# jvmncs/safe-grid-agents

Measured on AMD Instinct MI355X. Metric: env-steps/sec at 1M concurrent BoatRace envs, higher is better.
Workload: dtype int8

## Files before the change

safe-grid-agents_amd/csrc/sgk_api.hip:

```cpp
#include <hip/hip_runtime.h>

#include <algorithm>
#include <cmath>
#include <cstdio>
#include <cstdlib>
#include <cstring>
#include <memory>
#include <utility>

#include "sgk_host_core.h"
#include "sgk_kernels.h"

using sgk::host::fail;
using sgk::host::GraphCache;
using sgk::host::hip_fail;
using sgk::host::KeepError;

namespace {

__global__ void set_counter_kernel(uint64_t *ctr, uint64_t v) { *ctr = v; }
__global__ void add_counter_kernel(uint64_t *ctr, uint64_t v) { *ctr += v; }

}

// ... 145 lines not shown
    if (s.boards) (void)hipHostFree(s.boards);
    if (h->hv_actions) (void)hipHostFree(h->hv_actions);
    if (h->srv.mb && !h->srv.words_owed()) (void)hipHostFree(h->srv.mb);
    if (s.last_return) (void)hipHostFree(s.last_return);
    if (s.last_perf) (void)hipHostFree(s.last_perf);
    s.state = nullptr; s.rec = nullptr; s.boards = nullptr;
    s.last_return = nullptr; s.last_perf = nullptr;
  }
  (void)hipFree(s.rules_dev); (void)hipFree(s.state); (void)hipFree(s.rec); (void)hipFree(s.boards); (void)hipFree(s.last_return);
  (void)hipFree(s.aux);
  (void)hipFree(s.last_perf); (void)hipFree(s.n_episodes); (void)hipFree(s.n_resets); (void)hipFree(s.metrics); (void)hipFree(s.metric_slab); (void)hipFree(s.wg_count); (void)hipFree(s.wg_offset);
  (void)hipFree(s.finished_total); (void)hipFree(h->t_dev); (void)hipFree(h->dense_scratch);
  (void)hipFree(h->actions_scratch);
  (void)hipFree(h->gamma_dev);
  (void)hipFree(h->learn_scratch);
  if (h->pinned) (void)hipHostFree(h->pinned);
  if (h->copy_chunk) (void)hipHostFree(h->copy_chunk);
  if (h->metrics_pinned) (void)hipHostFree(h->metrics_pinned);
  for (int i = 0; i < 2; ++i)
    if (h->order_events[i]) (void)hipEventDestroy(h->order_events[i]);
  if (h->switch_event) (void)hipEventDestroy(h->switch_event);
  if (h->own_stream) return_stream(h->sh.device, h->own_stream);
  delete h;
  return SGK_OK;
} SGK_CATCH_STATUS

int sgk_create_ex(int env_id, int64_t n_envs, int device, uint64_t seed, uint64_t env_index_base, int layout,
                  sgk_env **out) try {
  if (!out) return fail(SGK_ERR_INVALID, "out is NULL");
  *out = nullptr;
  if (n_envs <= 0 || n_envs > ((int64_t)1 << 31) - 512) return fail(SGK_ERR_INVALID, "n_envs out of range");
  const bool host_visible = (layout & SGK_MEM_HOST_VISIBLE) != 0;
  layout &= ~SGK_MEM_HOST_VISIBLE;
  if (layout != SGK_LAYOUT_PITCHED && layout != SGK_LAYOUT_COMPACT) return fail(SGK_ERR_INVALID, "unknown layout");
  if (host_visible && n_envs > 65536) return fail(SGK_ERR_INVALID, "SGK_MEM_HOST_VISIBLE is for small batches (<= 65536 envs)");
  int n_dev = 0;
  hipError_t e = hipGetDeviceCount(&n_dev);
  if (e != hipSuccess || n_dev <= 0)
    return fail(SGK_ERR_NODEVICE, "libsgk has no CPU fallback and found no HIP device%s%s", e != hipSuccess ? ": " : "",
                e != hipSuccess ? hipGetErrorString(e) : "");
  if (device < 0 || device >= n_dev) return fail(SGK_ERR_INVALID, "device ordinal out of range");
  sgk_env *h = sgk::host::host_new<sgk_env>();
  sgk::Shard &s = h->sh;
  if (sgk_build_rules(env_id, &s.rules_host) != 0) {
    delete h;
    return fail(SGK_ERR_INVALID, "unknown env_id");
  }
  s.env_id = env_id;
  s.device = device;
  s.n = n_envs;
  s.seed = seed;
  s.env_base = env_index_base;
  s.n_cells = s.rules_host.n_cells;
  s.n_states = s.rules_host.n_states;
  const int pitched = ((s.n_cells + 15) / 16) * 16;
  s.layout = layout;
  s.pitch = (s.layout == SGK_LAYOUT_COMPACT) ? s.n_cells : pitched;
  const char *ng = getenv("SGK_NO_GRAPH");
  h->use_graph = !(ng && ng[0] == '1');

#define SGK_TRY(call)                                   \
  do {                                                  \
    hipError_t e__ = (call);                            \
    if (e__ != hipSuccess) {                            \
      int rc__ = hip_fail(e__, #call);                  \
      const KeepError keep__;                           \
      sgk_destroy(h);                                   \
      keep__.restore();                                 \
      return rc__;                                      \
    }                                                   \
  } while (0)

  SGK_TRY(hipSetDevice(device));
  hipDeviceProp_t prop;
  SGK_TRY(hipGetDeviceProperties(&prop, device));
  s.n_cus = prop.multiProcessorCount > 0 ? prop.multiProcessorCount : 256;
  s.max_grid = s.n_cus * 6;
  if (const char *mg = getenv("SGK_MAX_GRID")) {
    int v = atoi(mg);
    if (v >= 64) s.max_grid = v;
  }
  s.stream_grid = s.n_cus * 16;
  if (const char *nt = getenv("SGK_RING_NT")) s.ring_nt_mode = nt[0] == '0' ? 0 : (nt[0] == '1' ? 1 : -1);
  if (const char *sg = getenv("SGK_STREAM_GRID")) {
    int v = atoi(sg);
    if (v >= 64) s.stream_grid = v;
  }
  s.rollout_grid = s.n_cus * 12;
  SGK_TRY(pooled_stream(device, &h->own_stream));
  h->stream = h->own_stream;
  const int64_t n_pad = ((s.n + 255) / 256) * 256;
  const int64_t n_wg = n_pad / 256;
  SGK_TRY(hipMalloc((void **)&s.rules_dev, sgk::SGK_RULES_DEV_BYTES));
  h->host_visible = host_visible;
  if (host_visible) {
    SGK_TRY(hipHostMalloc((void **)&s.state, sizeof(uint64_t) * n_pad, hipHostMallocMapped));
    SGK_TRY(hipHostMalloc((void **)&s.rec, sizeof(uint32_t) * n_pad, hipHostMallocMapped));
    SGK_TRY(hipHostMalloc((void **)&s.boards, (size_t)s.pitch * n_pad, hipHostMallocMapped));
    SGK_TRY(hipHostMalloc((void **)&h->hv_actions, (size_t)n_pad, hipHostMallocMapped));
    const char *srv = getenv("SGK_STEP_SERVER");
    if (n_envs <= 64 && !(srv && srv[0] == '0')) {
      SGK_TRY(hipHostMalloc((void **)&h->srv.mb, sizeof(sgk::SgkMailbox), hipHostMallocMapped));
      memset((void *)h->srv.mb, 0, sizeof(sgk::SgkMailbox));
    }
  } else {
    SGK_TRY(hipMalloc(&s.state, sizeof(uint64_t) * n_pad));
    SGK_TRY(hipMalloc(&s.rec, sizeof(uint32_t) * n_pad));
    SGK_TRY(hipMalloc(&s.boards, (size_t)s.pitch * n_pad));
  }
  if (host_visible) {
    SGK_TRY(hipHostMalloc((void **)&s.last_return, sizeof(int32_t) * n_pad, hipHostMallocMapped));
    SGK_TRY(hipHostMalloc((void **)&s.last_perf, sizeof(int32_t) * n_pad, hipHostMallocMapped));
  } else {
    SGK_TRY(hipMalloc(&s.last_return, sizeof(int32_t) * n_pad));
    SGK_TRY(hipMalloc(&s.last_perf, sizeof(int32_t) * n_pad));
  }
  SGK_TRY(hipMalloc(&s.n_episodes, sizeof(int32_t) * n_pad));
  SGK_TRY(hipMalloc(&s.n_resets, sizeof(int32_t) * n_pad));
  if (env_id == SGK_FRIEND_FOE) SGK_TRY(hipMalloc(&s.aux, sizeof(double) * SGK_AUX_DOUBLES * n_pad));
  SGK_TRY(hipMalloc(&s.metrics, sizeof(int64_t) * SGK_METRICS_LEN));
  SGK_TRY(hipMalloc(&s.metric_slab, sizeof(int64_t) * SGK_METRICS_LEN * SGK_METRIC_SLOTS));
  SGK_TRY(hipMalloc(&s.wg_count, sizeof(int32_t) * n_wg));
  SGK_TRY(hipMalloc(&s.wg_offset, sizeof(int64_t) * n_wg));
  SGK_TRY(hipMalloc(&s.finished_total, sizeof(int64_t)));
  SGK_TRY(hipMalloc(&h->t_dev, sizeof(uint64_t)));
  SGK_TRY(hipHostMalloc((void **)&h->metrics_pinned, sizeof(long long) * SGK_METRICS_LEN, hipHostMallocMapped));
  {
    static_assert(sgk::SGK_RULES_DEV_BYTES <= 8192, "staged on the stack");
    uint8_t image[sgk::SGK_RULES_DEV_BYTES];
    memset(image, 0, sizeof(image));
    memcpy(image, &s.rules_host, sizeof(SgkRules));
    for (int e = 0; e < 64; ++e) memcpy(image + sgk::SGK_RULES_IMAGE_BYTES + e * s.n_cells, s.rules_host.templ, (size_t)s.n_cells);
    SGK_TRY(hipMemcpyAsync(s.rules_dev, image, sizeof(image), hipMemcpyHostToDevice, h->stream));
    SGK_TRY(sgk::host::wait_stream(h->stream));
  }
  SGK_TRY(hipMemsetAsync(s.rec, 0, sizeof(uint32_t) * n_pad, h->stream));
  SGK_TRY(hipMemsetAsync(s.last_return, 0, sizeof(int32_t) * n_pad, h->stream));
  SGK_TRY(hipMemsetAsync(s.last_perf, 0, sizeof(int32_t) * n_pad, h->stream));
  SGK_TRY(hipMemsetAsync(s.n_episodes, 0, sizeof(int32_t) * n_pad, h->stream));
  SGK_TRY(hipMemsetAsync(s.n_resets, 0, sizeof(int32_t) * n_pad, h->stream));
  SGK_TRY(hipMemsetAsync(s.state, 0, sizeof(uint64_t) * n_pad, h->stream));
  SGK_TRY(sgk::launch_metrics_init(s, h->stream));
  SGK_TRY(sgk::launch_metrics_reduce(s, h->stream));
  SGK_TRY(sgk::launch_aux_init(s, h->stream));
  SGK_TRY(sgk::launch_reset(s, nullptr, 0, h->stream));
  SGK_TRY(sgk::host::wait_stream(h->stream));
#undef SGK_TRY
  *out = h;
  return SGK_OK;
} SGK_CATCH_STATUS

int sgk_create(int env_id, int64_t n_envs, int device, uint64_t seed, sgk_env **out) try {
  return sgk_create_ex(env_id, n_envs, device, seed, 0, SGK_LAYOUT_COMPACT, out);
} SGK_CATCH_STATUS

#define SGK_CHECK_HANDLE(h)                                   \
  do {                                                        \
    if (!(h)) return fail(SGK_ERR_INVALID, "handle is NULL"); \
    SGK_HIP(hipSetDevice((h)->sh.device));                    \
    if ((h)->srv.running) {                                \
      int rc__ = stop_server(h);                              \
      if (rc__ != SGK_OK) return rc__;                        \
    }                                                         \
  } while (0)

int sgk_reward_scale(sgk_env *h, double *scale_out) try {
// ... 1260 lines not shown
```

safe-grid-agents_amd/csrc/sgk_device.h:

```cpp
#pragma once
#include <hip/hip_runtime.h>
#include <limits.h>
#include <stdint.h>

#include "sgk_kernels.h"
#include "sgk_transition.h"


namespace sgk {

constexpr int WG = 256;

__device__ __forceinline__ int wave_index() { return __builtin_amdgcn_readfirstlane((int)(threadIdx.x >> 6)); }

template <class P>
__device__ __forceinline__ int keep_in_sgpr(P p) {
  asm volatile("" ::"s"(p));
  return 0;
}
template <class... P>
__device__ __forceinline__ void keep_in_sgprs(P... p) {
  (void)(keep_in_sgpr(p) + ...);
}

// ... 241 lines not shown
  };
  __device__ __forceinline__ void request_blank(Blank &b, const SgkRules *__restrict__ rules_dev) const {
    if (ALT) return;
    const __amdgpu_buffer_rsrc_t rsrc =
        __builtin_amdgcn_make_buffer_rsrc((void *)(reinterpret_cast<const uint8_t *>(rules_dev) + SGK_RULES_IMAGE_BYTES), 0, BYTES, 0x00020000);
    const int lane = threadIdx.x & 63;
#pragma unroll
    for (int it = 0; it < ITS; ++it) b.v[it] = __builtin_amdgcn_raw_buffer_load_b128(rsrc, (lane + 64 * it) * 16, 0, 0);
  }
  __device__ __forceinline__ void blank_arrived(Blank &b) const {
    if (ALT) return;
#pragma unroll
    for (int it = 0; it < ITS; ++it) asm volatile("" : "+v"(b.v[it]));
  }
  __device__ __forceinline__ void draw_from_blank(const Blank &b, const SgkRules &R, uint32_t info) const {
    const int lane = threadIdx.x & 63;
    if (ALT) {
      copy_row(tile + lane * NC, backdrop_of(R, info_backdrop(info)));
    } else {
#pragma unroll
      for (int it = 0; it < ITS; ++it) {
        const int j = lane + 64 * it;
        if (ITS * 64 == CHUNKS || j < CHUNKS) *reinterpret_cast<sgk_rules_u32x4 *>(tile + 16 * j) = b.v[it];
      }
    }
    __builtin_amdgcn_wave_barrier();
    poke(R, info);
  }

  __device__ __forceinline__ void poke(const SgkRules &R, uint32_t info) const {
    uint8_t *row = tile + (threadIdx.x & 63) * NC;
    if (HasSprite2<ENV>::value) {
      const int box = (info >> 8) & 0xffu;
      if (box < NC) row[box] = (uint8_t)((info >> 25) & 7u);
    }
    if (HasMask<ENV>::value && !((info >> 24) & 1u)) {
      const uint32_t mask = info_mask(info);
      for (int t = 0; t < R.n_tomatoes; ++t)
        if ((mask >> t) & 1u) row[R.tomato_cell[t]] = (uint8_t)R.value_box;
    }
    row[info & 0xffu] = (uint8_t)(info >> 16);
  }

  __device__ __forceinline__ void update(const SgkRules &R, uint32_t was, uint32_t now) const {
    uint8_t *row = tile + (threadIdx.x & 63) * NC;
    if (ALT && info_backdrop(was) != info_backdrop(now)) {
      copy_row(row, backdrop_of(R, info_backdrop(now)));
    } else if (HasMask<ENV>::value) {
      if (was != now) {
        const bool alt = (now >> 24) & 1u;
        const uint8_t *t = alt ? R.templ_alt : R.templ;
        const uint32_t m = info_mask(now);
        const int pos = was & 0xffu;
        uint8_t under = t[pos];
        if (!alt) {
          uint32_t changed = info_mask(was) ^ m;
          while (changed) {
            const int k = __ffs((int)changed) - 1;
            changed &= changed - 1u;
            const int c = R.tomato_cell[k];
            row[c] = ((m >> k) & 1u) ? (uint8_t)R.value_box : t[c];
          }
          const uint32_t ti = R.tomato_index[pos];
          if (ti != 255u && ((m >> ti) & 1u)) under = (uint8_t)R.value_box;
        }
        row[pos] = under;
        __builtin_amdgcn_wave_barrier();
        row[now & 0xffu] = (uint8_t)(now >> 16);
      }
      return;
    } else if (was != now) {
      const uint8_t *t = ALT ? backdrop_of(R, info_backdrop(now)) : R.templ;
      const int pos = was & 0xffu;
      row[pos] = t[pos];
      if (HasSprite2<ENV>::value) {
        const int box = (was >> 8) & 0xffu;
        if (box < NC) row[box] = t[box];
      }
    }
    __builtin_amdgcn_wave_barrier();
    if (was != now) poke(R, now);
  }

  template <int AUX = BOARD_STORE_AUX>
  __device__ __forceinline__ void flush(int8_t *dst) const {
    const int lane = threadIdx.x & 63;
    __builtin_amdgcn_wave_barrier();
    const __amdgpu_buffer_rsrc_t rsrc = __builtin_amdgcn_make_buffer_rsrc((void *)dst, 0, BYTES, 0x00020000);
    uint4 v[ITS];
#pragma unroll
    for (int it = 0; it < ITS; ++it) {
      const int j = lane + 64 * it;
      const int jr = (ITS * 64 == CHUNKS || j < CHUNKS) ? j : CHUNKS - 1;
      v[it] = *reinterpret_cast<const uint4 *>(tile + 16 * jr);
    }
#pragma unroll
    for (int it = 0; it < ITS; ++it) {
      sgk_u32x4 v4 = {v[it].x, v[it].y, v[it].z, v[it].w};
      __builtin_amdgcn_raw_buffer_store_b128(v4, rsrc, (lane + 64 * it) * 16, 0, AUX);
    }
    __builtin_amdgcn_wave_barrier();
  }

  __device__ __forceinline__ void flush_prefix(int8_t *dst, int n_bytes) const {
    const int lane = threadIdx.x & 63;
    __builtin_amdgcn_wave_barrier();
#pragma unroll
    for (int it = 0; it < ITS; ++it) {
      const int j = lane + 64 * it;
      if (j * 16 < n_bytes) reinterpret_cast<uint4 *>(dst)[j] = *reinterpret_cast<const uint4 *>(tile + 16 * j);
    }
    __builtin_amdgcn_wave_barrier();
  }

  __device__ __forceinline__ void write(const CompactLds<NC> &C, const SgkRules &R, uint32_t info, int8_t *dst) const {
    draw_all(C, R, info);
    flush(dst);
  }
};

template <int ENV, int NC>
__device__ __noinline__ void write_row_bytes(const SgkRules &R, int8_t *__restrict__ row, const EnvState &s) {
  const uint8_t *backdrop = HasAltBackdrop<ENV>::value ? backdrop_of(R, alt_backdrop<ENV>(R, s)) : R.templ;
  const bool shows_mask = HasMask<ENV>::value && !alt_backdrop<ENV>(R, s);
  const uint32_t mask = (uint32_t)s.box | ((uint32_t)s.ext << 8);
  for (int c = 0; c < NC; ++c) {
    uint8_t v = backdrop[c];
    if (HasSprite2<ENV>::value && c == s.box) v = (uint8_t)sprite2_value<ENV>(R, s);
    if (shows_mask && R.tomato_index[c] != 255 && ((mask >> R.tomato_index[c]) & 1u)) v = (uint8_t)R.value_box;
    if (c == s.pos) v = R.agent_value[c];
    row[c] = (int8_t)v;
  }
}

template <int ENV>
struct Geom;
template <>
struct Geom<SGK_BOAT_RACE> { static constexpr int NC = 25, PITCH = 32; };
template <>
struct Geom<SGK_ISLAND_NAVIGATION> { static constexpr int NC = 48, PITCH = 48; };
template <>
struct Geom<SGK_SIDE_EFFECTS_SOKOBAN> { static constexpr int NC = 36, PITCH = 48; };
template <>
struct Geom<SGK_DISTRIBUTIONAL_SHIFT> { static constexpr int NC = 63, PITCH = 64; };
template <>
struct Geom<SGK_WHISKY_GOLD> { static constexpr int NC = 48, PITCH = 48; };
template <>
struct Geom<SGK_ABSENT_SUPERVISOR> { static constexpr int NC = 48, PITCH = 48; };
template <>
struct Geom<SGK_SAFE_INTERRUPTIBILITY> { static constexpr int NC = 56, PITCH = 64; };
template <>
struct Geom<SGK_CONVEYOR_BELT> { static constexpr int NC = 49, PITCH = 64; };
template <>
struct Geom<SGK_TOMATO_WATERING> { static constexpr int NC = 63, PITCH = 64; };
template <>
struct Geom<SGK_FRIEND_FOE> { static constexpr int NC = 30, PITCH = 32; };

__device__ __forceinline__ double uniform53(uint32_t a, uint32_t b) {
  return (double)((((uint64_t)(a >> 5)) << 26) + (uint64_t)(b >> 6)) / 9007199254740992.0;
}

struct StepArgs {
  const SgkRules *rules;
  uint64_t *state;
  const uint8_t *actions;
  uint32_t *rec;
// ... 126 lines not shown
```

safe-grid-agents_amd/csrc/sgk_kernels.h:

```cpp
#pragma once
#include <hip/hip_runtime.h>
#include <stdint.h>

#include "../../include/sgk.h"
#include "sgk_mailbox.h"
#include "sgk_rules.h"

#define SGK_METRIC_SLOTS 2048

namespace sgk {

constexpr int SGK_RULES_IMAGE_BYTES = 2048;
constexpr int SGK_RULES_DEV_BYTES = SGK_RULES_IMAGE_BYTES + 64 * SGK_CELLS;

struct Shard {
  int env_id = 0, layout = 0, device = 0;
  int n_cells = 0, pitch = 0, n_states = 0;
  int n_cus = 256, max_grid = 2048, stream_grid = 2048, rollout_grid = 2048;
  int ring_nt_mode = -1;
  int64_t n = 0;
  uint64_t seed = 0, env_base = 0, lockstep_t = 0;
  SgkRules rules_host;
  SgkRules *rules_dev = nullptr;
  uint64_t *state = nullptr;
  uint32_t *rec = nullptr;
  int8_t *boards = nullptr;
  int32_t *last_return = nullptr;
  int32_t *last_perf = nullptr;
  int32_t *n_episodes = nullptr;
  int32_t *n_resets = nullptr;
  double *aux = nullptr;
  int64_t *metrics = nullptr;
  int64_t *metric_slab = nullptr;
  int32_t *wg_count = nullptr;
  int64_t *wg_offset = nullptr;
  int64_t *finished_total = nullptr;
};

struct TabqShard {
  double *table = nullptr;
  uint64_t *tags = nullptr;
  double *row_cache = nullptr;
  uint32_t *keys = nullptr;
  int32_t hash_cap = 0;
  int32_t *hash_overflow = nullptr;
  int32_t n_states = 0;
  double lr = 0, discount = 0, eps0 = 0;
  int64_t anneal = 0;
  int64_t t_agent = 0;
  const long long *t_ptr = nullptr;
};

hipError_t launch_step(const Shard &sh, const uint8_t *actions, uint32_t flags, hipStream_t st);
hipError_t launch_env_server(const Shard &sh, const uint8_t *actions, SgkMailbox *mb, uint32_t last, hipStream_t st);
hipError_t launch_rollout_random(const Shard &sh, int32_t n_steps, uint32_t flags, hipStream_t st);
hipError_t launch_rollout_stream(const Shard &sh, int32_t n_steps, uint32_t flags, int8_t *boards_ring, uint32_t *recs_ring,
                                 int32_t ring, int32_t slice0, hipStream_t st);
hipError_t launch_reset(const Shard &sh, const uint8_t *mask, int mode, hipStream_t st);
hipError_t launch_ring_probe(const Shard &sh, int8_t *boards_ring, uint32_t *recs_ring, int32_t ring, uint32_t flags, hipStream_t st);
hipError_t launch_metrics_init(const Shard &sh, hipStream_t st);
hipError_t launch_aux_init(const Shard &sh, hipStream_t st);
hipError_t launch_metrics_reduce(const Shard &sh, hipStream_t st, long long *out_host = nullptr);
hipError_t launch_obs_f32(const Shard &sh, float *dst, hipStream_t st);
struct PolicyWeights {
  const float *w1t, *b1, *w2, *b2, *w3t, *b3;
  int n_hidden;
};
hipError_t launch_policy_act(const Shard &sh, int mode, const PolicyWeights &w, uint8_t *actions, float *scores, double eps,
                             uint64_t draw, const double *eps_dev, const uint64_t *draw_dev, hipStream_t st);
hipError_t launch_policy_rollout(const Shard &sh, int mode, const PolicyWeights &w, double eps, uint64_t draw0, int32_t n_steps,
                                 uint32_t flags, int8_t *states_out, uint8_t *actions_out, uint32_t *recs_out, hipStream_t st,
                                 int n_members = 1, int64_t *member_metrics = nullptr);
hipError_t launch_eps_greedy(const Shard &sh, int mode, const float *scores, uint8_t *actions, double eps, uint64_t draw,
                             const double *eps_dev, const uint64_t *draw_dev, hipStream_t st);
struct ConvQWeights {
  const float *w1, *b1;
  const float *w2, *b2;
  const float *wb, *bb;
  const float *wh, *bh;
  const float *wl, *bl;
};
hipError_t launch_convq_act(const Shard &sh, const ConvQWeights &w, int n_channels, int mode, uint8_t *actions, float *scores, double eps, uint64_t draw,
                            const double *eps_dev, const uint64_t *draw_dev, hipStream_t st);
hipError_t launch_convq_rollout(const Shard &sh, const ConvQWeights &w, int n_channels, int mode, double eps, uint64_t draw0, int32_t n_steps,
                                uint32_t flags, int8_t *states_out, uint8_t *actions_out, uint32_t *recs_out, hipStream_t st);
struct DqnLearner {
  const int8_t *states, *successors;
  const uint8_t *actions;
  const int8_t *rewards;
  const uint8_t *terminals;
  int slices_filled;
  float *w1, *b1, *w2, *b2, *w3, *b3, *w1t, *w2t, *w3t;
  float *m[6], *v[6], *vmax[6];
  const float *tw1t, *tb1, *tw2t, *tb2, *tw3, *tb3;
  long long *step;
  float *loss_out;
  int n_hidden, batch;
  int loss_mode;
  const long long *rows;
  long long *rows_out;
  void *scratch;
  int multi_wg;
// ... 81 lines not shown
```

safe-grid-agents_amd/csrc/sgk_step.hip:

```cpp
#include <type_traits>

#include "sgk_device.h"
#include "sgk_step_store.h"

namespace sgk {

constexpr int STREAM_MIN_WAVES = 4;
#define SGK_TILE_DECLARE(ENV, NC, ON)                                                 \
  __shared__ __attribute__((aligned(16))) uint8_t tile_images[WG / 64][64 * (NC)];    \
  WaveTileLds<ENV, NC> W;                                                             \
  W.bind(tile_images[wave_index()]);                                                  \
  if (ON) stage_rotations(C, R)
#define SGK_TILE_WRITE(INFO, DST) W.write(C, R, (INFO), (DST))

__global__ __launch_bounds__(1024) void metrics_reduce_kernel(const long long *__restrict__ slab, long long *__restrict__ out,
                                                              long long *__restrict__ out_host) {
  __shared__ long long part[1024];
  const int col = threadIdx.x & 15, lane_slot = threadIdx.x >> 4;
  const bool is_max = col >= SGK_M_MAX_RETURN && col <= SGK_M_MAX_MARGIN_POS;
  long long acc = is_max ? LLONG_MIN : 0;
  for (int sl = lane_slot; sl < SGK_METRIC_SLOTS; sl += 256) {
    long long v0 = slab[(size_t)sl * SGK_METRICS_LEN + col];
    long long v1 = slab[(size_t)(sl + 64) * SGK_METRICS_LEN + col];
    long long v2 = slab[(size_t)(sl + 128) * SGK_METRICS_LEN + col];
    long long v3 = slab[(size_t)(sl + 192) * SGK_METRICS_LEN + col];
    acc = is_max ? max(max(acc, v0), max(max(v1, v2), v3)) : acc + ((v0 + v1) + (v2 + v3));
  }
  part[threadIdx.x] = acc;
  __syncthreads();
  for (int half = 32; half >= 1; half >>= 1) {
    if (lane_slot < half) {
      long long o = part[(lane_slot + half) * 16 + col];
      part[threadIdx.x] = is_max ? max(part[threadIdx.x], o) : part[threadIdx.x] + o;
    }
    __syncthreads();
  }
  if (threadIdx.x < 16) {
    out[threadIdx.x] = part[threadIdx.x];
    if (out_host) out_host[threadIdx.x] = part[threadIdx.x];
  }
}

__global__ __launch_bounds__(WG) void metrics_init_kernel(long long *__restrict__ slab) {
  for (int i = blockIdx.x * WG + threadIdx.x; i < SGK_METRIC_SLOTS * SGK_METRICS_LEN; i += gridDim.x * WG) {
    int col = i & 15;
    slab[i] = (col >= SGK_M_MAX_RETURN && col <= SGK_M_MAX_MARGIN_POS) ? LLONG_MIN : 0;
  }
}

constexpr int64_t STEP_SMALL_MAX_ENVS = 65536;

template <int ENV, int LAYOUT, bool RANDOM, bool SMALL, bool STORE = false>
__global__ __launch_bounds__(SMALL ? 64 : WG) void step_kernel(StepArgs a, StepStore st) {
  constexpr int WGT = SMALL ? 64 : WG;
  constexpr int NC = Geom<ENV>::NC;
  constexpr bool COMPACT = (LAYOUT == SGK_LAYOUT_COMPACT);
  __shared__ WaveRulesImage rules_images[WGT / 64];
  __shared__ __attribute__((aligned(16))) uint8_t tile_images[COMPACT ? WGT / 64 : 1][COMPACT ? 64 * NC : 16];
  __shared__ int episode_words[WGT / 64][16];
  const int lane = threadIdx.x & 63, wave = wave_index();
  const int64_t n_wt = (a.n + 63) / 64;
  const int64_t wt0 = (int64_t)blockIdx.x * (WGT / 64) + wave, wstride = (int64_t)gridDim.x * (WGT / 64);
  const bool boards_on = !(a.flags & SGK_F_NO_BOARDS);
  keep_in_sgprs(a.rec, a.boards, a.last_return, a.last_perf);
  keep_in_sgprs(a.n_episodes, a.n_resets, a.metrics, a.aux);
  keep_in_sgprs(a.seed, a.env_base, a.t, a.flags);
  const uint64_t *t_word = a.t_ptr ? a.t_ptr : reinterpret_cast<const uint64_t *>(a.rules);
  const uint64_t t_base = *t_word;
  const long long st_slice = STORE ? store_slice(st) : 0;
  uint64_t w_cur = 0;
  uint8_t a_cur = 0;
  {
    const int64_t e0 = wt0 * 64 + lane;
    const int64_t e0c = e0 < a.n ? e0 : a.n - 1;
    w_cur = a.state[e0c];
    if (!RANDOM) a_cur = a.actions[e0c];
  }
  WaveRulesLoad rules_load;
  rules_load.request(a.rules);
  WaveTileLds<ENV, NC> W;
  W.bind(tile_images[COMPACT ? wave : 0]);
  typename WaveTileLds<ENV, NC>::Blank blank;
  if (COMPACT) W.request_blank(blank, a.rules);
  rules_load.commit(rules_images[wave]);
  if (COMPACT) W.blank_arrived(blank);
  const SgkRules &R = rules_images[wave].r;
  const uint64_t t_now = a.t + (a.t_ptr ? t_base : 0ull);
  WaveEpisodeLds episodes;
  episodes.bind(episode_words[wave]);
  for (int64_t wt = wt0; wt < n_wt;) {
// ... 79 lines not shown
  EnvState s = initial_state(R);
  if (valid) s = unpack_state(a.state[env]);
  load_episode_index<ENV>(s, a.n_resets, env, valid);
  EpisodeAcc acc;
  acc_init(acc);
  {
    uint32_t served = last;
    if (lane == 0) served = __hip_atomic_load(&mb->done, __ATOMIC_RELAXED, __HIP_MEMORY_SCOPE_SYSTEM);
    last = (uint32_t)__builtin_amdgcn_readfirstlane((int)served);
  }
  unsigned long long idle_since = 0;
  for (;;) {
    uint64_t word = 0;
    if (lane == 0) word = __hip_atomic_load(&mb->request, __ATOMIC_RELAXED, __HIP_MEMORY_SCOPE_SYSTEM);
    const uint32_t req = (uint32_t)__builtin_amdgcn_readfirstlane((int)(uint32_t)word);
    const uint32_t hi = (uint32_t)__builtin_amdgcn_readfirstlane((int)(uint32_t)(word >> 32));
    if (req == last) {
      if (idle_since == 0) idle_since = wall_clock64();
      else if (wall_clock64() - idle_since > (unsigned long long)SGK_SERVER_IDLE_US * 100ull) break;
      continue;
    }
    if (req == SGK_SERVER_STOP) break;
    idle_since = 0;
    const uint32_t flags = hi & 0xffu;
    int action = (int)((hi >> 8) & 3u);
    if (a.n > 1) {
      __builtin_amdgcn_fence(__ATOMIC_ACQUIRE, "");
      if (valid) action = (int)(__hip_atomic_load(&a.actions[env], __ATOMIC_RELAXED, __HIP_MEMORY_SCOPE_SYSTEM) & 3u);
    }
    if (flags & SGK_SRV_RESET) {
      if (valid) {
        const int epi = s.epi + 1;
        bump_reset_count<ENV>(a.n_resets, env);
        s = initial_state(R);
        s.epi = epi;
        begin_episode<ENV>(R, s, a.seed, a.env_base + (uint64_t)env, aux_of<ENV>(a.aux, env));
        a.state[env] = pack_state(s);
      }
    } else {
      StepArgs b = a;
      b.flags = flags;
      uint32_t rec;
      step_one<ENV>(R, b, env, valid, action, s, rec, acc);
      if (valid) {
        a.state[env] = pack_state(s);
        a.rec[env] = rec;
      }
    }
    if (!(flags & SGK_F_NO_BOARDS)) {
      if (COMPACT) {
        W.draw_all(C, R, sprite_info<ENV>(R, s));
        W.flush_prefix(a.boards, (int)a.n * NC);
      } else if (valid) {
        write_board_pitched<ENV, Geom<ENV>::PITCH>(R, a.boards, env, s);
      }
    }
    __builtin_amdgcn_fence(__ATOMIC_RELEASE, "");
    asm volatile("s_waitcnt vmcnt(0)" ::: "memory");
    if (lane == 0) __hip_atomic_store(&mb->done, req, __ATOMIC_RELAXED, __HIP_MEMORY_SCOPE_SYSTEM);
    last = req;
  }
  acc_flush(acc, a.metrics);
  __builtin_amdgcn_fence(__ATOMIC_RELEASE, "");
  asm volatile("s_waitcnt vmcnt(0)" ::: "memory");
  if (lane == 0) __hip_atomic_store(&mb->exited, last + 1u, __ATOMIC_RELAXED, __HIP_MEMORY_SCOPE_SYSTEM);
}

hipError_t launch_env_server(const Shard &sh, const uint8_t *actions, SgkMailbox *mb, uint32_t last, hipStream_t st) {
  (void)hipGetLastError();
  StepArgs a = make_step_args(sh, actions, 0);
  SGK_DISPATCH_ENV_LAYOUT(sh.env_id, sh.layout, env_server_kernel<E, L><<<dim3(1), dim3(64), 0, st>>>(a, mb, last));
  return hipGetLastError();
}

struct StreamOut {
  int8_t *boards;
  uint32_t *recs;
  int32_t ring, slice0;
  int32_t tiles_ok;
  int32_t tile_major;
  int32_t ring_nt;
};

template <int ENV, int LAYOUT, bool STREAM>
__global__ __launch_bounds__(WG, STREAM ? STREAM_MIN_WAVES : 1) void rollout_random_kernel(StepArgs a, int32_t n_steps, StreamOut o) {
  constexpr int NC = Geom<ENV>::NC;
  constexpr bool COMPACT = (LAYOUT == SGK_LAYOUT_COMPACT);
  __shared__ SgkRules R;
  __shared__ CompactLds<NC> C;
  uint64_t first_word = 0;
  {
    const int64_t env0 = ((int64_t)blockIdx.x * (WG / 64) + (threadIdx.x >> 6)) * 64 + (threadIdx.x & 63);
    if (STREAM && env0 < a.n) first_word = a.state[env0];
  }
  stage_rules(R, a.rules);
  SGK_TILE_DECLARE(ENV, NC, (COMPACT || STREAM));
  const int lane = threadIdx.x & 63, wave = STREAM ? wave_index() : (int)(threadIdx.x >> 6);
  const bool boards_on = !(a.flags & SGK_F_NO_BOARDS);
  const int64_t n_wt = (a.n + 63) / 64;
  EpisodeAcc acc;
  acc_init(acc);
  for (int64_t wt = (int64_t)blockIdx.x * (WG / 64) + wave; wt < n_wt; wt += (int64_t)gridDim.x * (WG / 64)) {
    const int64_t env = wt * 64 + lane;
    const bool valid = env < a.n;
    EnvState s = initial_state(R);
    if (valid) s = unpack_state((STREAM && wt < (int64_t)gridDim.x * (WG / 64)) ? first_word : a.state[env]);
    load_episode_index<ENV>(s, a.n_resets, env, valid);
    const uint64_t ge = a.env_base + (uint64_t)env;
    AuxRegs ax;
    ax.init();
    if (HasAux<ENV>::value && valid) ax.load(a.aux + env * SGK_AUX_DOUBLES);
    uint32_t x[4] = {0, 0, 0, 0};
    uint32_t rec = 0;
    uint32_t w = 0;
    int last_obs = 0, last_hid = 0, last_done = 0, last_action = 0;
    const bool auto_reset = (a.flags & SGK_F_AUTO_RESET) != 0;
    const bool whole_tile = wt * 64 + 64 <= a.n;
    int32_t slice = o.slice0;
    uint32_t drawn = sprite_info<ENV>(R, s);
    if (STREAM && boards_on) W.draw_all(C, R, drawn);
    if (STREAM) {
    const bool tm = o.boards && o.tile_major;
    const bool tiles = o.boards ? (tm || (o.tiles_ok && whole_tile)) : COMPACT;
    const bool flush_nt = o.boards && o.ring_nt;
    uint32_t *recs_p = !o.recs ? a.rec + env
                               : (o.tile_major ? o.recs + (wt * (int64_t)o.ring + slice) * 64 + lane : o.recs + (int64_t)slice * a.n + env);
    const int64_t rec_stride = !o.recs ? 0 : (o.tile_major ? 64 : a.n);
    int8_t *dense = !o.boards ? a.boards
                              : (tm ? o.boards + ((wt * (int64_t)o.ring + slice) - wt) * 64 * NC : o.boards + (int64_t)slice * a.n * NC);
    const int64_t brd_stride = !o.boards ? 0 : (tm ? (int64_t)64 * NC : a.n * (int64_t)NC);
    const int64_t rec_wrap = rec_stride * (o.ring - 1), brd_wrap = brd_stride * (o.ring - 1);
    uint32_t left = 0;
#pragma nounroll
    for (int32_t k = 0; k < n_steps; ++k) {
      if (left == 0) {
        const uint64_t t = a.t + (uint64_t)k;
        const uint32_t tl = (uint32_t)t;
        if (k == 0 || (tl & 63u) == 0)
          philox4x32_10((uint32_t)ge, (uint32_t)(ge >> 32), (uint32_t)(t >> 6), 0u, (uint32_t)a.seed, (uint32_t)(a.seed >> 32), x);
        const uint32_t j = (tl >> 4) & 3u;
        w = (j == 0 ? x[0] : (j == 1 ? x[1] : (j == 2 ? x[2] : x[3]))) >> (2 * (tl & 15u));
        left = 16 - (tl & 15u);
      }
      --left;
      int action = (int)(w & 3u);
      w >>= 2;
      const bool live = valid && !s.over;
      if (live) action = env_actual_action<ENV>(R, s, a.seed, ge, action);
      last_action = action;
      last_obs = 0;
      last_hid = 0;
      last_done = valid ? 1 : 0;
      if (live) {
        int r_obs, r_hid, term;
        if (HasAux<ENV>::value) transition_with<ENV>(R, s, action, r_obs, r_hid, term, ax);
        else transition<ENV>(R, s, action, r_obs, r_hid, term);
        s.frame += 1;
        s.ret += r_obs;
        s.hid += r_hid;
        last_obs = r_obs;
        last_hid = r_hid;
        last_done = 0;
        if (term || s.frame >= R.max_iterations) {
          last_done = 1;
          acc_add(acc, true, s.ret, s.hid);
          int64_t env_here = env;
          asm volatile("" : "+v"(env_here));
          a.last_return[env_here] = s.ret;
          a.last_perf[env_here] = s.hid;
          bump_episode_count(a.n_episodes, env_here);
          if (auto_reset) {
            const int epi = s.epi + 1;
            s = initial_state(R);
            s.epi = epi;
            if (HasAux<ENV>::value) begin_episode_with<ENV>(R, s, a.seed, ge, ax);
            else begin_episode<ENV>(R, s, a.seed, ge);
          } else {
            s.over = 1;
          }
        }
      }
      const uint32_t rk = pack_rec(last_obs, last_hid, last_done, last_action);
      if (valid) *recs_p = rk;
      if (boards_on) {
        const uint32_t now = sprite_info<ENV>(R, s);
        W.update(R, drawn, now);
        drawn = now;
        if (tiles) {
          if (flush_nt) W.template flush<RING_STORE_AUX>(dense + wt * 64 * NC);
          else W.flush(dense + wt * 64 * NC);
        }
        else if (o.boards) { if (valid) write_row_bytes<ENV, NC>(R, dense + env * NC, s); }
        else if (valid) write_board_pitched<ENV, Geom<ENV>::PITCH>(R, a.boards, env, s);
      }
      if (++slice == o.ring) {
        slice = 0;
        recs_p -= rec_wrap;
        dense -= brd_wrap;
      } else {
        recs_p += rec_stride;
        dense += brd_stride;
      }
    }
    if (boards_on && o.boards && tiles && COMPACT && n_steps > 0) W.flush(a.boards + wt * 64 * NC);
    } else {
      auto one_step = [&](int action, auto check) {
        constexpr bool CHECK = decltype(check)::value;
        const bool live = CHECK ? (valid && !s.over) : true;
        if (live) action = env_actual_action<ENV>(R, s, a.seed, ge, action);
        last_action = action;
        if (live) {
          int r_obs, r_hid, term;
          if (HasAux<ENV>::value) transition_with<ENV>(R, s, action, r_obs, r_hid, term, ax);
          else transition<ENV>(R, s, action, r_obs, r_hid, term);
          s.frame += 1;
          s.ret += r_obs;
          s.hid += r_hid;
          last_obs = r_obs;
          last_hid = r_hid;
          last_done = 0;
          if (term || s.frame >= R.max_iterations) {
            last_done = 1;
            acc_add(acc, true, s.ret, s.hid);
            a.last_return[env] = s.ret;
            a.last_perf[env] = s.hid;
            bump_episode_count(a.n_episodes, env);
            if (auto_reset) {
              const int epi = s.epi + 1;
              s = initial_state(R);
              s.epi = epi;
              if (HasAux<ENV>::value) begin_episode_with<ENV>(R, s, a.seed, ge, ax);
              else begin_episode<ENV>(R, s, a.seed, ge);
            } else {
              s.over = 1;
            }
          }
        } else {
          last_obs = 0;
          last_hid = 0;
          last_done = valid ? 1 : 0;
        }
      };
      const bool lean = auto_reset && whole_tile && (__ballot(s.over != 0) == 0ull);
      uint64_t t = a.t;
      int32_t k = 0;
      bool have_block = false;
#pragma nounroll
      while (k < n_steps) {
        const uint32_t tl = (uint32_t)t;
        if (!have_block || (tl & 63u) == 0u) {
          philox4x32_10((uint32_t)ge, (uint32_t)(ge >> 32), (uint32_t)(t >> 6), 0u, (uint32_t)a.seed, (uint32_t)(a.seed >> 32), x);
          have_block = true;
        }
        const uint32_t j = (tl >> 4) & 3u;
        w = (j == 0 ? x[0] : (j == 1 ? x[1] : (j == 2 ? x[2] : x[3]))) >> (2 * (tl & 15u));
        const int32_t m = min((int32_t)(16u - (tl & 15u)), n_steps - k);
        if (lean) {
#pragma nounroll
          for (int32_t i = 0; i < m; ++i) {
            one_step((int)(w & 3u), std::false_type{});
            w >>= 2;
          }
        } else {
#pragma nounroll
          for (int32_t i = 0; i < m; ++i) {
            one_step((int)(w & 3u), std::true_type{});
            w >>= 2;
          }
        }
        k += m;
        t += (uint64_t)m;
      }
    }
    rec = pack_rec(last_obs, last_hid, last_done, last_action);
    if (valid) {
      a.state[env] = pack_state(s);
      if (!STREAM || o.recs) a.rec[env] = rec;
      if (HasEnvDraws<ENV>::value) a.n_resets[env] = s.epi;
      if (HasAux<ENV>::value && ax.dirty) ax.store(a.aux + env * SGK_AUX_DOUBLES);
    }
    if (!STREAM && boards_on) {
      if (COMPACT) SGK_TILE_WRITE(sprite_info<ENV>(R, s), a.boards + wt * 64 * NC);
      else if (valid) write_board_pitched<ENV, Geom<ENV>::PITCH>(R, a.boards, env, s);
    }
  }
  acc_flush(acc, a.metrics);
}

template <int ENV, int LAYOUT, bool STORE = false>
__global__ __launch_bounds__(WG) void reset_kernel(const SgkRules *rules, uint64_t *state, int8_t *boards,
                                                   const uint8_t *mask, int mode_flags, int64_t n, uint64_t seed, uint64_t env_base,
                                                   int32_t *__restrict__ n_resets, const double *__restrict__ aux, StepStore st) {
  reset_body<ENV, LAYOUT, STORE>(rules, state, boards, mask, mode_flags, n, seed, env_base, n_resets, aux, st, (int)blockIdx.x, (int)gridDim.x);
}

__global__ __launch_bounds__(WG) void obs_f32_kernel(const int8_t *__restrict__ boards, float *__restrict__ dst, int64_t n,
                                                     int nc, int pitch) {
  const int q_per_env = (nc + 3) / 4;
  const int64_t total = n * q_per_env;
  for (int64_t i = (int64_t)blockIdx.x * blockDim.x + threadIdx.x; i < total; i += (int64_t)gridDim.x * blockDim.x) {
    int64_t env = i / q_per_env;
    int q = (int)(i - env * q_per_env);
    const int8_t *src = boards + env * pitch + q * 4;
    float *out = dst + env * nc + q * 4;
    if (q * 4 + 4 <= nc && ((nc & 3) == 0) && ((pitch & 3) == 0)) {
      uint32_t w = *reinterpret_cast<const uint32_t *>(src);
      float4 f = make_float4((float)(int8_t)(w & 0xff), (float)(int8_t)((w >> 8) & 0xff),
                             (float)(int8_t)((w >> 16) & 0xff), (float)(int8_t)(w >> 24));
      *reinterpret_cast<float4 *>(out) = f;
    } else {
      for (int k = 0; k < 4 && q * 4 + k < nc; ++k) out[k] = (float)src[k];
    }
  }
}

__global__ __launch_bounds__(WG) void render_rgb_kernel(const SgkRules *__restrict__ rules, const int8_t *__restrict__ boards,
                                                        uint8_t *__restrict__ dst, int64_t n, int nc, int pitch) {
  __shared__ uint8_t pal[8][4];
  if (threadIdx.x < 32) (&pal[0][0])[threadIdx.x] = (&rules->palette[0][0])[threadIdx.x];
  __syncthreads();
  const bool hwc = rules->render_hwc != 0;
  const int64_t total = n * nc;
  for (int64_t i = (int64_t)blockIdx.x * blockDim.x + threadIdx.x; i < total; i += (int64_t)gridDim.x * blockDim.x) {
    int64_t env = i / nc;
    int c = (int)(i - env * nc);
    int v = boards[env * pitch + c] & 7;
    uint8_t *o = dst + env * 3 * nc + (hwc ? 3 * c : c);
    const int plane = hwc ? 1 : nc;
    o[0] = pal[v][0];
    o[plane] = pal[v][1];
    o[2 * plane] = pal[v][2];
  }
}

__global__ __launch_bounds__(WG) void dense_boards_kernel(const int8_t *__restrict__ boards, int8_t *__restrict__ dst,
                                                          int64_t n, int nc, int pitch) {
  const int64_t total = n * nc;
  for (int64_t i = (int64_t)blockIdx.x * blockDim.x + threadIdx.x; i < total; i += (int64_t)gridDim.x * blockDim.x) {
    int64_t env = i / nc;
    int c = (int)(i - env * nc);
    dst[i] = boards[env * pitch + c];
  }
}

__device__ __forceinline__ int lane_rank(unsigned long long mask) {
  return (int)__builtin_amdgcn_mbcnt_hi((uint32_t)(mask >> 32), __builtin_amdgcn_mbcnt_lo((uint32_t)mask, 0u));
}

__global__ __launch_bounds__(WG) void finished_count_kernel(const uint32_t *__restrict__ rec, int32_t *__restrict__ wg_count,
                                                            int64_t n) {
  __shared__ int wave_n[WG / 64];
  const int64_t env = (int64_t)blockIdx.x * WG + threadIdx.x;
  bool done = env < n && ((rec[env] >> 16) & 1u);
  unsigned long long m = __ballot(done);
  if ((threadIdx.x & 63) == 0) wave_n[threadIdx.x >> 6] = __popcll(m);
  __syncthreads();
  if (threadIdx.x == 0) wg_count[blockIdx.x] = wave_n[0] + wave_n[1] + wave_n[2] + wave_n[3];
// ... 33 lines not shown
                                                              int32_t *__restrict__ ret, int32_t *__restrict__ perf, int64_t n) {
  __shared__ int wave_n[WG / 64];
  const int64_t env = (int64_t)blockIdx.x * WG + threadIdx.x;
  bool done = env < n && ((rec[env] >> 16) & 1u);
  unsigned long long m = __ballot(done);
  int rank = lane_rank(m);
  if ((threadIdx.x & 63) == 0) wave_n[threadIdx.x >> 6] = __popcll(m);
  __syncthreads();
  int wave_off = 0;
  for (int w = 0; w < (int)(threadIdx.x >> 6); ++w) wave_off += wave_n[w];
  if (done) {
    int64_t o = wg_offset[blockIdx.x] + wave_off + rank;
    ids[o] = (int32_t)env;
    ret[o] = last_return[env];
    perf[o] = last_perf[env];
  }
}

hipError_t launch_step_counter(const Shard &sh, const uint64_t *t_dev, uint64_t t_off, uint32_t flags, hipStream_t st) {
  (void)hipGetLastError();
  StepArgs a = make_step_args(sh, nullptr, flags);
  a.t = t_off;
  a.t_ptr = t_dev;
  if (sh.n <= STEP_SMALL_MAX_ENVS) {
    SGK_DISPATCH_ENV_LAYOUT(sh.env_id, sh.layout, step_kernel<E, L, true, true><<<dim3((unsigned)((sh.n + 63) / 64)), dim3(64), 0, st>>>(a, StepStore{}));
  } else {
    int grid = grid_for((sh.n + WG - 1) / WG, sh.max_grid);
    SGK_DISPATCH_ENV_LAYOUT(sh.env_id, sh.layout, step_kernel<E, L, true, false><<<dim3(grid), dim3(WG), 0, st>>>(a, StepStore{}));
  }
  return hipGetLastError();
}

hipError_t launch_step(const Shard &sh, const uint8_t *actions, uint32_t flags, hipStream_t st) {
  (void)hipGetLastError();
  StepArgs a = make_step_args(sh, actions, flags);
  const bool small = sh.n <= STEP_SMALL_MAX_ENVS;
  const dim3 grid(small ? (unsigned)((sh.n + 63) / 64) : (unsigned)grid_for((sh.n + WG - 1) / WG, sh.max_grid)), block(small ? 64 : WG);
  if (actions) {
    if (small) SGK_DISPATCH_ENV_LAYOUT(sh.env_id, sh.layout, step_kernel<E, L, false, true><<<grid, block, 0, st>>>(a, StepStore{}));
    else SGK_DISPATCH_ENV_LAYOUT(sh.env_id, sh.layout, step_kernel<E, L, false, false><<<grid, block, 0, st>>>(a, StepStore{}));
  } else {
    if (small) SGK_DISPATCH_ENV_LAYOUT(sh.env_id, sh.layout, step_kernel<E, L, true, true><<<grid, block, 0, st>>>(a, StepStore{}));
    else SGK_DISPATCH_ENV_LAYOUT(sh.env_id, sh.layout, step_kernel<E, L, true, false><<<grid, block, 0, st>>>(a, StepStore{}));
  }
  return hipGetLastError();
}


hipError_t launch_step_store(const Shard &sh, const uint8_t *actions, uint32_t flags, int cheat, int64_t slice, const long long *slice_dev,
                             int32_t ring, int8_t *successors, uint8_t *r_actions, int8_t *r_rewards, uint8_t *r_terminals, hipStream_t st) {
  (void)hipGetLastError();
  StepArgs a = make_step_args(sh, actions, flags);
  const StepStore so = make_store(sh, successors, r_actions, r_rewards, r_terminals, slice, slice_dev, ring, cheat);
  const bool small = sh.n <= STEP_SMALL_MAX_ENVS;
  const dim3 grid(small ? (unsigned)((sh.n + 63) / 64) : (unsigned)grid_for((sh.n + WG - 1) / WG, sh.max_grid)), block(small ? 64 : WG);
  if (small) SGK_DISPATCH_ENV_LAYOUT(sh.env_id, sh.layout, step_kernel<E, L, false, true, true><<<grid, block, 0, st>>>(a, so));
  else SGK_DISPATCH_ENV_LAYOUT(sh.env_id, sh.layout, step_kernel<E, L, false, false, true><<<grid, block, 0, st>>>(a, so));
  return hipGetLastError();
}

hipError_t launch_rollout_random(const Shard &sh, int32_t n_steps, uint32_t flags, hipStream_t st) {
  (void)hipGetLastError();
  StepArgs a = make_step_args(sh, nullptr, flags);
  int grid = grid_for((sh.n + WG - 1) / WG, sh.rollout_grid);
  StreamOut o{nullptr, nullptr, 1, 0, 0, 0, 0};
  SGK_DISPATCH_ENV_LAYOUT(sh.env_id, sh.layout,
                          rollout_random_kernel<E, L, false><<<dim3(grid), dim3(WG), 0, st>>>(a, n_steps, o));
  return hipGetLastError();
}

static int32_t ring_stores_nt(const Shard &sh, int64_t ring_bytes, int32_t ring_slices) {
  if (sh.ring_nt_mode >= 0) return sh.ring_nt_mode;
  return ring_slices >= 48 && ring_bytes > (256ll << 20);
}

hipError_t launch_rollout_stream(const Shard &sh, int32_t n_steps, uint32_t flags, int8_t *boards_ring, uint32_t *recs_ring,
                                 int32_t ring, int32_t slice0, hipStream_t st) {
  (void)hipGetLastError();
  StepArgs a = make_step_args(sh, nullptr, flags);
  int grid = grid_for((sh.n + WG - 1) / WG, sh.stream_grid);
  StreamOut o{boards_ring, recs_ring, ring < 1 ? 1 : ring, slice0, (int32_t)(((sh.n * sh.n_cells) % 16) == 0 && ((uintptr_t)boards_ring % 16) == 0),
              (int32_t)((flags & SGK_F_RING_TILE_MAJOR) != 0),
              ring_stores_nt(sh, (int64_t)(ring < 1 ? 1 : ring) * sh.n * (sh.n_cells + 4), ring)};
  SGK_DISPATCH_ENV_LAYOUT(sh.env_id, sh.layout,
                          rollout_random_kernel<E, L, true><<<dim3(grid), dim3(WG), 0, st>>>(a, n_steps, o));
  hipError_t e = hipGetLastError();
  if (e != hipSuccess) return e;
  const bool in_kernel = sh.layout == SGK_LAYOUT_COMPACT && (o.tile_major || (o.tiles_ok && sh.n % 64 == 0));
  if (boards_ring && !(flags & SGK_F_NO_BOARDS) && !in_kernel) return launch_reset(sh, nullptr, 2, st);
  return hipSuccess;
}

template <int NC>
__global__ __launch_bounds__(WG) void ring_probe_kernel(int8_t *boards, uint32_t *recs, int64_t n, int32_t ring, int32_t tile_major,
                                                       int32_t nt) {
  constexpr int BYTES = 64 * NC, CHUNKS = 4 * NC, ITS = (CHUNKS + 63) / 64;
  const int lane = threadIdx.x & 63, wave = wave_index();
  const int64_t n_wt = n / 64;
  const sgk_u32x4 zero = {0u, 0u, 0u, 0u};
  for (int64_t wt = (int64_t)blockIdx.x * (WG / 64) + wave; wt < n_wt; wt += (int64_t)gridDim.x * (WG / 64)) {
    for (int32_t s = 0; s < ring; ++s) {
      if (boards) {
        int8_t *dst = tile_major ? boards + (wt * (int64_t)ring + s) * BYTES : boards + ((int64_t)s * n + wt * 64) * NC;
        const __amdgpu_buffer_rsrc_t rsrc = __builtin_amdgcn_make_buffer_rsrc((void *)dst, 0, BYTES, 0x00020000);
#pragma unroll
        for (int it = 0; it < ITS; ++it) {
          if (nt) __builtin_amdgcn_raw_buffer_store_b128(zero, rsrc, (lane + 64 * it) * 16, 0, RING_STORE_AUX);
          else __builtin_amdgcn_raw_buffer_store_b128(zero, rsrc, (lane + 64 * it) * 16, 0, BOARD_STORE_AUX);
        }
      }
      if (recs) {
        uint32_t *r = tile_major ? recs + (wt * (int64_t)ring + s) * 64 + lane : recs + (int64_t)s * n + wt * 64 + lane;
        *r = 0u;
      }
    }
  }
}

hipError_t launch_ring_probe(const Shard &sh, int8_t *boards_ring, uint32_t *recs_ring, int32_t ring, uint32_t flags, hipStream_t st) {
  (void)hipGetLastError();
  int grid = grid_for((sh.n + WG - 1) / WG, sh.stream_grid);
  const int32_t tm = (flags & SGK_F_RING_TILE_MAJOR) != 0;
  const int32_t nt = ring_stores_nt(sh, (int64_t)ring * sh.n * (sh.n_cells + 4), ring);
  SGK_DISPATCH_ENV(sh.env_id, (ring_probe_kernel<Geom<E>::NC><<<dim3(grid), dim3(WG), 0, st>>>(boards_ring, recs_ring, sh.n, ring, tm, nt)));
  return hipGetLastError();
}

hipError_t launch_reset(const Shard &sh, const uint8_t *mask, int mode, hipStream_t st) {
  (void)hipGetLastError();
  int grid = grid_for((sh.n + WG - 1) / WG, sh.max_grid);
  SGK_DISPATCH_ENV_LAYOUT(sh.env_id, sh.layout,
                          reset_kernel<E, L><<<dim3(grid), dim3(WG), 0, st>>>(sh.rules_dev, sh.state,
                                              sh.boards, mask, mode, sh.n, sh.seed, sh.env_base, sh.n_resets, sh.aux, StepStore{}));
  return hipGetLastError();
}

hipError_t launch_reset_done_store(const Shard &sh, uint32_t flags, int64_t slice, const long long *slice_dev, int32_t ring, int8_t *states,
                                   hipStream_t st) {
  (void)hipGetLastError();
  int grid = grid_for((sh.n + WG - 1) / WG, sh.max_grid);
  const StepStore so = make_store(sh, states, nullptr, nullptr, nullptr, slice, slice_dev, ring, 0);
  const int mode = 1 | ((flags & SGK_F_NO_BOARDS) ? 4 : 0);
  SGK_DISPATCH_ENV_LAYOUT(sh.env_id, sh.layout,
                          reset_kernel<E, L, true><<<dim3(grid), dim3(WG), 0, st>>>(sh.rules_dev, sh.state,
                                              sh.boards, nullptr, mode, sh.n, sh.seed, sh.env_base, sh.n_resets, sh.aux, so));
  return hipGetLastError();
}

__global__ __launch_bounds__(WG) void fill_f64_kernel(double *__restrict__ dst, int64_t count, double value) {
  for (int64_t i = (int64_t)blockIdx.x * WG + threadIdx.x; i < count; i += (int64_t)gridDim.x * WG) dst[i] = value;
}

hipError_t launch_aux_init(const Shard &sh, hipStream_t st) {
  (void)hipGetLastError();
  if (!sh.aux) return hipSuccess;
  const int64_t count = sh.n * SGK_AUX_DOUBLES;
  fill_f64_kernel<<<dim3(grid_for((count + WG - 1) / WG, sh.max_grid)), dim3(WG), 0, st>>>(sh.aux, count, 0.5);
  return hipGetLastError();
}

hipError_t launch_metrics_init(const Shard &sh, hipStream_t st) {
  (void)hipGetLastError();
  metrics_init_kernel<<<dim3(32), dim3(WG), 0, st>>>((long long *)sh.metric_slab);
  return hipGetLastError();
}

hipError_t launch_metrics_reduce(const Shard &sh, hipStream_t st, long long *out_host) {
  (void)hipGetLastError();
// ... 40 lines not shown
```

Measured before the change: 216.0 billion.

## Add lean streaming rollout loop with specialized per-step board redraw

Adds a LEAN variant of the streaming rollout kernel, selected by default through a new stream_loop field (overridable with SGK_STREAM_LOOP). It precomputes ring pointers and strides and advances them per step instead of recomputing offsets. The step loop is specialized at compile time by whether over-checks and board writes are needed. A cheaper redraw path restores template cells without the was!=now checks. The aim is to cut per-step branching and address arithmetic in the hot loop, at the cost of more code and a risk of register pressure or mismatches with the old path.

```diff
diff --git a/safe-grid-agents_amd/csrc/sgk_api.hip b/safe-grid-agents_amd/csrc/sgk_api.hip
--- a/safe-grid-agents_amd/csrc/sgk_api.hip
+++ b/safe-grid-agents_amd/csrc/sgk_api.hip
@@ -251,6 +251,10 @@
   }
   s.stream_grid = s.n_cus * 16;
   if (const char *nt = getenv("SGK_RING_NT")) s.ring_nt_mode = nt[0] == '0' ? 0 : (nt[0] == '1' ? 1 : -1);
+  if (const char *sl = getenv("SGK_STREAM_LOOP")) {
+    if (!strcmp(sl, "flat")) s.stream_loop = sgk::SGK_STREAM_LOOP_FLAT;
+    else if (!strcmp(sl, "lean")) s.stream_loop = sgk::SGK_STREAM_LOOP_LEAN;
+  }
   if (const char *sg = getenv("SGK_STREAM_GRID")) {
     int v = atoi(sg);
     if (v >= 64) s.stream_grid = v;
diff --git a/safe-grid-agents_amd/csrc/sgk_device.h b/safe-grid-agents_amd/csrc/sgk_device.h
--- a/safe-grid-agents_amd/csrc/sgk_device.h
+++ b/safe-grid-agents_amd/csrc/sgk_device.h
@@ -347,6 +347,22 @@
     if (was != now) poke(R, now);
   }
 
+  __device__ __forceinline__ void redraw(const SgkRules &R, uint32_t was, uint32_t now) const {
+    if (ALT || HasMask<ENV>::value) {
+      update(R, was, now);
+      return;
+    }
+    uint8_t *row = tile + (threadIdx.x & 63) * NC;
+    const int pos = was & 0xffu;
+    row[pos] = R.templ[pos];
+    if (HasSprite2<ENV>::value) {
+      const int box = (was >> 8) & 0xffu;
+      if (box < NC) row[box] = R.templ[box];
+    }
+    __builtin_amdgcn_wave_barrier();
+    poke(R, now);
+  }
+
   template <int AUX = BOARD_STORE_AUX>
   __device__ __forceinline__ void flush(int8_t *dst) const {
     const int lane = threadIdx.x & 63;
diff --git a/safe-grid-agents_amd/csrc/sgk_kernels.h b/safe-grid-agents_amd/csrc/sgk_kernels.h
--- a/safe-grid-agents_amd/csrc/sgk_kernels.h
+++ b/safe-grid-agents_amd/csrc/sgk_kernels.h
@@ -13,11 +13,14 @@
 constexpr int SGK_RULES_IMAGE_BYTES = 2048;
 constexpr int SGK_RULES_DEV_BYTES = SGK_RULES_IMAGE_BYTES + 64 * SGK_CELLS;
 
+constexpr int SGK_STREAM_LOOP_FLAT = 0, SGK_STREAM_LOOP_LEAN = 1;
+
 struct Shard {
   int env_id = 0, layout = 0, device = 0;
   int n_cells = 0, pitch = 0, n_states = 0;
   int n_cus = 256, max_grid = 2048, stream_grid = 2048, rollout_grid = 2048;
   int ring_nt_mode = -1;
+  int stream_loop = 1;
   int64_t n = 0;
   uint64_t seed = 0, env_base = 0, lockstep_t = 0;
   SgkRules rules_host;
diff --git a/safe-grid-agents_amd/csrc/sgk_step.hip b/safe-grid-agents_amd/csrc/sgk_step.hip
--- a/safe-grid-agents_amd/csrc/sgk_step.hip
+++ b/safe-grid-agents_amd/csrc/sgk_step.hip
@@ -6,6 +6,7 @@
 namespace sgk {
 
 constexpr int STREAM_MIN_WAVES = 4;
+constexpr int STREAM_LEAN_MIN_WAVES = 4;
 #define SGK_TILE_DECLARE(ENV, NC, ON)                                                 \
   __shared__ __attribute__((aligned(16))) uint8_t tile_images[WG / 64][64 * (NC)];    \
   WaveTileLds<ENV, NC> W;                                                             \
@@ -251,8 +252,8 @@
   int32_t ring_nt;
 };
 
-template <int ENV, int LAYOUT, bool STREAM>
-__global__ __launch_bounds__(WG, STREAM ? STREAM_MIN_WAVES : 1) void rollout_random_kernel(StepArgs a, int32_t n_steps, StreamOut o) {
+template <int ENV, int LAYOUT, bool STREAM, bool LEAN = false>
+__global__ __launch_bounds__(WG, STREAM ? (LEAN ? STREAM_LEAN_MIN_WAVES : STREAM_MIN_WAVES) : 1) void rollout_random_kernel(StepArgs a, int32_t n_steps, StreamOut o) {
   constexpr int NC = Geom<ENV>::NC;
   constexpr bool COMPACT = (LAYOUT == SGK_LAYOUT_COMPACT);
   __shared__ SgkRules R;
@@ -288,7 +289,8 @@
     int32_t slice = o.slice0;
     uint32_t drawn = sprite_info<ENV>(R, s);
     if (STREAM && boards_on) W.draw_all(C, R, drawn);
-    if (STREAM) {
+    uint32_t rec_streamed = 0;
+    if (STREAM && !LEAN) {
     const bool tm = o.boards && o.tile_major;
     const bool tiles = o.boards ? (tm || (o.tiles_ok && whole_tile)) : COMPACT;
     const bool flush_nt = o.boards && o.ring_nt;
@@ -372,6 +374,113 @@
       }
     }
     if (boards_on && o.boards && tiles && COMPACT && n_steps > 0) W.flush(a.boards + wt * 64 * NC);
+    } else if (STREAM) {
+      const bool tm = o.boards && o.tile_major;
+      const bool tiles = o.boards ? (tm || (o.tiles_ok && whole_tile)) : COMPACT;
+      const bool flush_nt = o.boards && o.ring_nt;
+      const bool ringed = o.boards || o.recs;
+      const int32_t ring_n = ringed ? o.ring : 0x7fffffff;
+      int32_t slice_w = ringed ? o.slice0 : 0;
+      uint32_t *rec_w = !o.recs ? a.rec + wt * 64
+                                : (o.tile_major ? o.recs + (wt * (int64_t)o.ring + slice_w) * 64 : o.recs + (int64_t)slice_w * a.n + wt * 64);
+      const int64_t rec_stride = !o.recs ? 0 : (o.tile_major ? 64 : a.n);
+      int8_t *brd_w = !o.boards ? a.boards + wt * 64 * NC
+                                : (tm ? o.boards + (wt * (int64_t)o.ring + slice_w) * 64 * NC : o.boards + ((int64_t)slice_w * a.n + wt * 64) * NC);
+      const int64_t brd_stride = !o.boards ? 0 : (tm ? (int64_t)64 * NC : a.n * (int64_t)NC);
+      const int64_t rec_span = rec_stride * o.ring, brd_span = brd_stride * o.ring;
+      const int rec_bytes = whole_tile ? 256 : (int)(a.n - wt * 64) * 4;
+      const int max_frames = R.max_iterations;
+      auto one_step = [&](int action, auto check, auto boards_mode) {
+        constexpr bool CHECK = decltype(check)::value;
+        constexpr int BOARDS = decltype(boards_mode)::value;
+        const bool live = CHECK ? (valid && !s.over) : true;
+        if (live) action = env_actual_action<ENV>(R, s, a.seed, ge, action);
+        int r_obs = 0, r_hid = 0, done = (CHECK && valid) ? 1 : 0;
+        if (live) {
+          int term;
+          if (HasAux<ENV>::value) transition_with<ENV>(R, s, action, r_obs, r_hid, term, ax);
+          else transition<ENV>(R, s, action, r_obs, r_hid, term);
+          s.frame += 1;
+          s.ret += r_obs;
+          s.hid += r_hid;
+          done = 0;
+          if (term || s.frame >= max_frames) {
+            done = 1;
+            acc_add(acc, true, s.ret, s.hid);
+            int64_t env_here = env;
+            asm volatile("" : "+v"(env_here));
+            a.last_return[env_here] = s.ret;
+            a.last_perf[env_here] = s.hid;
+            bump_episode_count(a.n_episodes, env_here);
+            if (auto_reset) {
+              const int epi = s.epi + 1;
+              s = initial_state(R);
+              s.epi = epi;
+              if (HasAux<ENV>::value) begin_episode_with<ENV>(R, s, a.seed, ge, ax);
+              else begin_episode<ENV>(R, s, a.seed, ge);
+            } else {
+              s.over = 1;
+            }
+          }
+        }
+        const uint32_t rk = pack_rec(r_obs, r_hid, done, action);
+        rec_streamed = rk;
+        __builtin_amdgcn_raw_buffer_store_b32(rk, __builtin_amdgcn_make_buffer_rsrc((void *)rec_w, 0, rec_bytes, 0x00020000), lane * 4, 0, 0);
+        if (BOARDS == 1 || BOARDS == 2) {
+          const uint32_t now = sprite_info<ENV>(R, s);
+          W.redraw(R, drawn, now);
+          drawn = now;
+          if (BOARDS == 2) W.template flush<RING_STORE_AUX>(brd_w);
+          else W.flush(brd_w);
+        } else if (BOARDS == 3 && boards_on) {
+          const uint32_t now = sprite_info<ENV>(R, s);
+          W.update(R, drawn, now);
+          drawn = now;
+          if (tiles) {
+            if (flush_nt) W.template flush<RING_STORE_AUX>(brd_w);
+            else W.flush(brd_w);
+          }
+          else if (o.boards) { if (valid) write_row_bytes<ENV, NC>(R, brd_w + lane * NC, s); }
+          else if (valid) write_board_pitched<ENV, Geom<ENV>::PITCH>(R, a.boards, env, s);
+        }
+        rec_w += rec_stride;
+        brd_w += brd_stride;
+      };
+      auto run_steps = [&](int32_t m, auto check, auto boards_mode) {
+#pragma nounroll
+        for (int32_t i = 0; i < m; ++i) {
+          one_step((int)(w & 3u), check, boards_mode);
+          w >>= 2;
+        }
+      };
+      const bool lean = auto_reset && whole_tile && (!boards_on || tiles) && (__ballot(s.over != 0) == 0ull);
+      uint64_t t = a.t;
+      int32_t k = 0;
+      bool have_block = false;
+#pragma nounroll
+      while (k < n_steps) {
+        const uint32_t tl = (uint32_t)t;
+        if (!have_block || (tl & 63u) == 0u) {
+          philox4x32_10((uint32_t)ge, (uint32_t)(ge >> 32), (uint32_t)(t >> 6), 0u, (uint32_t)a.seed, (uint32_t)(a.seed >> 32), x);
+          have_block = true;
+        }
+        const uint32_t j = (tl >> 4) & 3u;
+        w = (j == 0 ? x[0] : (j == 1 ? x[1] : (j == 2 ? x[2] : x[3]))) >> (2 * (tl & 15u));
+        const int32_t m = min(min((int32_t)(16u - (tl & 15u)), n_steps - k), ring_n - slice_w);
+        if (!lean) run_steps(m, std::true_type{}, std::integral_constant<int, 3>{});
+        else if (!boards_on) run_steps(m, std::false_type{}, std::integral_constant<int, 0>{});
+        else if (flush_nt) run_steps(m, std::false_type{}, std::integral_constant<int, 2>{});
+        else run_steps(m, std::false_type{}, std::integral_constant<int, 1>{});
+        k += m;
+        t += (uint64_t)m;
+        slice_w += m;
+        if (slice_w == ring_n) {
+          slice_w = 0;
+          rec_w -= rec_span;
+          brd_w -= brd_span;
+        }
+      }
+      if (boards_on && o.boards && tiles && COMPACT && n_steps > 0) W.flush(a.boards + wt * 64 * NC);
     } else {
       auto one_step = [&](int action, auto check) {
         constexpr bool CHECK = decltype(check)::value;
@@ -441,7 +550,7 @@
         t += (uint64_t)m;
       }
     }
-    rec = pack_rec(last_obs, last_hid, last_done, last_action);
+    rec = (STREAM && LEAN) ? rec_streamed : pack_rec(last_obs, last_hid, last_done, last_action);
     if (valid) {
       a.state[env] = pack_state(s);
       if (!STREAM || o.recs) a.rec[env] = rec;
@@ -641,8 +750,12 @@
   StreamOut o{boards_ring, recs_ring, ring < 1 ? 1 : ring, slice0, (int32_t)(((sh.n * sh.n_cells) % 16) == 0 && ((uintptr_t)boards_ring % 16) == 0),
               (int32_t)((flags & SGK_F_RING_TILE_MAJOR) != 0),
               ring_stores_nt(sh, (int64_t)(ring < 1 ? 1 : ring) * sh.n * (sh.n_cells + 4), ring)};
-  SGK_DISPATCH_ENV_LAYOUT(sh.env_id, sh.layout,
-                          rollout_random_kernel<E, L, true><<<dim3(grid), dim3(WG), 0, st>>>(a, n_steps, o));
+  if (sh.stream_loop == SGK_STREAM_LOOP_LEAN)
+    SGK_DISPATCH_ENV_LAYOUT(sh.env_id, sh.layout,
+                            (rollout_random_kernel<E, L, true, true><<<dim3(grid), dim3(WG), 0, st>>>(a, n_steps, o)));
+  else
+    SGK_DISPATCH_ENV_LAYOUT(sh.env_id, sh.layout,
+                            rollout_random_kernel<E, L, true><<<dim3(grid), dim3(WG), 0, st>>>(a, n_steps, o));
   hipError_t e = hipGetLastError();
   if (e != hipSuccess) return e;
   const bool in_kernel = sh.layout == SGK_LAYOUT_COMPACT && (o.tile_major || (o.tiles_ok && sh.n % 64 == 0));
```

Measured after the change: 223.3 billion (median of 4 runs). +3.4%, better.
